# prabhask5/real-time-ray-tracing-engine

Hardware: AMD Instinct MI355X
Metric: Msamples/sec (W×H×spp) at 1080p, 8-bounce; 1/2/4/8 MI355X + CPU ref (higher is better)
Workload: dtype f64; 1 GPU; C2 three_spheres 1920x1080 spp64 depth8; scene=three_spheres, width=1920, height=1080, spp=64, max_depth=8, parallelism=1 GPU, device=gpu

## Files before the change

### __graft_entry__.py

```python
import os
import subprocess
import sys

ROOT = os.path.dirname(os.path.abspath(__file__))
PKG = os.path.join(ROOT, "real-time-ray-tracing-engine_amd")


def _make(path, *targets):
    jobs = "-j%d" % min(16, os.cpu_count() or 1)
    subprocess.run(["make", jobs, "-C", path] + list(targets), check=True)


def build():
    _make(PKG)
    _make(os.path.join(ROOT, "oracle"))
    _make(os.path.join(ROOT, "tests", "native"))
    _make(os.path.join(ROOT, "tests", "native"), "-f", "guides.mk")
    _make(os.path.join(ROOT, "tests", "native"), "-f", "temporal.mk")
    _make(os.path.join(ROOT, "tests", "native"), "-f", "temporal_variance.mk")
    _make(os.path.join(ROOT, "tests", "native"), "-f", "root_table.mk")
    _make(os.path.join(ROOT, "tests", "native"), "-f", "diffuse.mk")
    _make(os.path.join(ROOT, "tests", "native"), "-f", "unitv.mk")
    _make(os.path.join(ROOT, "tests", "native"), "-f", "refit.mk")
    _make(os.path.join(ROOT, "tests", "native"), "-f", "live.mk")
    _make(os.path.join(ROOT, "tests", "native"), "-f", "query.mk")
    _make(os.path.join(ROOT, "tests", "native"), "-f", "occlusion.mk")
    _make(os.path.join(ROOT, "tests", "native"), "-f", "lambert.mk")
    _make(os.path.join(ROOT, "tests", "native"), "-f", "radiance.mk")
    if os.path.isdir("/root/reference/src"):
        _make(os.path.join(ROOT, "oracle"), "ref")
    for p in (PKG, os.path.join(ROOT, "tests")):
        if p not in sys.path:
            sys.path.insert(0, p)
    import rtx
    from rtx.lib import load
    load()


def smoke():
    for p in (PKG, os.path.join(ROOT, "tests")):
        if p not in sys.path:
            sys.path.insert(0, p)
    import numpy as np
    import torch
    from rtx.render import Renderer, camera_frame
    from rtx.scene import load_scene
    import oracle_lib as O

    assert torch.cuda.is_available(), "smoke() needs a GPU"
    S = load_scene(os.path.join(PKG, "scenes", "cornell_fog.json"))
    cam = S.camera_desc(image_width=32, samples_per_pixel=4, max_depth=8)
    f = camera_frame(cam)
    with Renderer(S, device=0) as R:
        gpu = R.render(f, seed=42)
    ref = O.oracle_render(S, cam, O.MODE_COUNTER, 42)
    d = float(np.nanmax(np.abs(gpu - ref)))
    assert d <= 1e-4, "GPU vs oracle max |diff| %g" % d
    print("smoke ok: %dx%d cornell_fog, max |gpu - oracle| = %.3g" % (f.image_width, f.image_height, d))


if __name__ == "__main__":
    build()
    if len(sys.argv) > 1 and sys.argv[1] == "smoke":
        smoke()
```

### real-time-ray-tracing-engine_amd/csrc/rt_camq.h

```cpp
#ifndef RT_CAMQ_H
#define RT_CAMQ_H

#if defined(__HIPCC__)
#include <hip/hip_runtime.h>
#define RT_CAMQ_HD __host__ __device__
#else
#define RT_CAMQ_HD
#endif

namespace rtq {

constexpr int kBatch = 64;
constexpr int kBatches = 2;
constexpr int kEntries = kBatch * kBatches;
constexpr int kComps = 7;

RT_CAMQ_HD inline int camq_need(int next_item, int n_idle, int n_items) {
  const int e = next_item + n_idle;
  return e < n_items ? e : n_items;
}
RT_CAMQ_HD inline bool camq_generate(int gen_items, int need) { return gen_items < need; }
RT_CAMQ_HD inline int camq_batch(int gen_items) { return gen_items / kBatch; }
RT_CAMQ_HD inline int camq_write_entry(int gen_items, int lane) { return (gen_items & (kEntries - 1)) + lane; }
RT_CAMQ_HD inline int camq_read_entry(int item) { return item & (kEntries - 1); }
RT_CAMQ_HD inline bool camq_may_overwrite(int gen_items, int next_item) {
  return gen_items < kEntries || next_item >= gen_items - kBatch;
}

}
#endif
```

### real-time-ray-tracing-engine_amd/csrc/rt_kernel.hip

```cpp
#include <hip/hip_runtime.h>
#include <stdint.h>
#include <stdlib.h>

#include <algorithm>
#include <array>
#include <mutex>
#include <set>
#include <utility>

#include "rt_camq.h"
#include "rt_kernels.h"
#include "rt_lds_plan.h"
#include "rt_path.h"
#include "rt_plan.h"

namespace {

using namespace rtp;
#ifndef RT_REGEN_FLAT
#define RT_REGEN_FLAT 16
#endif
#define RT_REGEN_MIN(F) ((F) == F_FLAT ? RT_REGEN_FLAT : (((F) & ~F_BVH4) == 0 ? 16 : 1))
#ifndef RT_PARK_K
#define RT_PARK_K 48
// ... 164 lines not shown
      const bool whole = S.n_lds_nodes >= S.n_nodes;
      for (int k = threadIdx.x; k < n8; k += blockDim.x) {
        const int i = k / 10, j = k - 10 * (k / 10);
        const int a = j / 3, m = j - 3 * (j / 3);
        const int u = j == 9 ? 6 : (m == 1 ? 3 + a : a);
        uint2 v = src[8 * i + u];
        if (j == 9 && whole) {
          if ((int)v.x >= 0) v.x *= (unsigned)sizeof(DNodeL);
          if ((int)v.y >= 0) v.y *= (unsigned)sizeof(DNodeL);
        }
        dst[k] = v;
      }
    }
    if constexpr (PC) {
      if (S.lds_items_pc > 0) {
        const int ni = S.lds_items_pc * 2, ns = S.lds_spheres_pc * 4;
        const int4 *si = reinterpret_cast<const int4 *>(S.items);
        const int4 *ss = reinterpret_cast<const int4 *>(S.spheres);
        for (int k = threadIdx.x; k < ni; k += blockDim.x) prim_g[k] = si[k];
        for (int k = threadIdx.x; k < ns; k += blockDim.x) prim_g[ni + k] = ss[k];
      }
    }
    __syncthreads();
  }
  if constexpr ((F & F_NOISE) != 0) {
    if (S.lds_perlin) {
      const int4 *src = reinterpret_cast<const int4 *>(S.perlin);
      RT_LDS int4 *dst = (RT_LDS int4 *)perlin_lds();
      for (int k = threadIdx.x; k < (int)(sizeof(DPerlin) / 16); k += blockDim.x) dst[k] = src[k];
      __syncthreads();
    }
  }
  const int n_units = P.n_head * P.head_chunks + (P.n_local_tiles - P.n_head) * P.n_chunks;
  int unit = blockIdx.x * BW + wv;
  int *stk = stack_base + wv * S.stack_depth * 64 + lane;
  double *acc = &acc_lds[wv][0][0];
  Counters cnt{0, 0, 0, 0, 0, 0, 0, 0, 0, 0, 0, 0, 0, 0, 0};
  uint64_t cyc_regen = 0;
  const uint64_t t_start = STATS ? clk() : 0;
  uint32_t n_samples = 0, n_segments = 0, n_trips = 0;
  uint64_t m_single = 0, m_pair = 0;
  uint32_t v_prev = 0, m_prev = 0;
  bool have_prev = false;
  auto wave_max = [](uint32_t x) {
    for (int off = 32; off > 0; off >>= 1) x = max(x, (uint32_t)__shfl_xor((int)x, off));
    return x;
  };
  while (unit < n_units) {
#if RT_UNIT_TIMES
  const unsigned long long t_unit0 = __builtin_amdgcn_s_memrealtime();
#endif
  const DLaunch PU = launch_fields<PC>(P);
  const int head_units = PU.n_head * PU.head_chunks;
  const bool whole = PU.head_chunks == 1 && unit < PU.n_head;
  int local_tile, s_first, s_count;
  {
    const bool head = unit < head_units;
    const int nc = head ? PU.head_chunks : PU.n_chunks;
    const int cs = head ? (PU.sample_count + nc - 1) / nc : PU.chunk_strata;
    const int u = head ? unit : unit - head_units, q = u / nc, chunk = u - q * nc;
    local_tile = head ? q : PU.n_head + q;
    s_first = PU.sample_begin + chunk * cs;
    s_count = min(cs, PU.sample_count - chunk * cs);
  }
  local_tile = order_tile(PU, local_tile);
  if constexpr (STATS || COST) {
    if (lane == 0 && PU.tile_cost != nullptr)
      atomicSub(&PU.tile_cost[local_tile], (unsigned)__builtin_amdgcn_s_memrealtime());
  }
  const int tile = PU.tile_first + local_tile * PU.tile_stride;
  const int tx = tile % PU.tiles_x, ty = tile / PU.tiles_x;
  const int x0 = tx * 8, y0 = PU.row_begin + ty * 8;
  acc[lane * 3 + 0] = 0.0;
  acc[lane * 3 + 1] = 0.0;
  acc[lane * 3 + 2] = 0.0;

  const int n_items = 64 * max(0, s_count);
  int next_item = 0;
  constexpr bool kCamq = F == F_FLAT;
  [[maybe_unused]] int gen_items = 0;
  PathState ps;
  ps.active = false;
  Key key{P.seed_lo, P.seed_hi, 0, 0};
  constexpr int kPark = RT_PARK_MIN(F);
  [[maybe_unused]] double pk_closest = 0.0;
  [[maybe_unused]] int pk_best = -1;

  for (;;) {
    const uint64_t t_regen = STATS ? clk() : 0;
    for (;;) {
      unsigned long long idle = __ballot(!ps.active);
      if (idle == 0 || next_item >= n_items) break;
      if (__popcll(idle) < RT_REGEN_MIN(F) && ~idle != 0ull) break;
      if constexpr (kCamq) {
        static_assert(BW == 1, "the camera-ray queue is one wave's");
        __shared__ double camq[rtq::kComps][rtq::kEntries];
        const DCamera &Cr = C;
        const bool lens = !(Cr.defocus_angle <= 0);
        const int rank = (int)__builtin_amdgcn_mbcnt_hi((uint32_t)(idle >> 32), __builtin_amdgcn_mbcnt_lo((uint32_t)idle, 0u));
        const int item = next_item + rank;
        const int need = __builtin_amdgcn_readfirstlane(rtq::camq_need(next_item, __popcll(idle), n_items));
        while (rtq::camq_generate(gen_items, need)) {
          const DCamera Cg = camera_fields<true>(C);
          const int gk = __builtin_amdgcn_readfirstlane(s_first + rtq::camq_batch(gen_items));
          const int gi = x0 + (lane & 7), gj = y0 + (lane >> 3);
          const Key gkey{P.seed_lo, P.seed_hi, (uint32_t)(gj * Cg.W + gi), (uint32_t)gk};
          const Ray gr = camera_ray<RT_KB_F(F), RT_KCONST_MODE(F)>(Cg, gkey, gi, gj, gk);
          const int e = rtq::camq_write_entry(gen_items, lane);
          camq[0][e] = gr.d.x;
          camq[1][e] = gr.d.y;
          camq[2][e] = gr.d.z;
          camq[3][e] = gr.tm;
          if (lens) {
            camq[4][e] = gr.o.x;
            camq[5][e] = gr.o.y;
            camq[6][e] = gr.o.z;
          }
          gen_items += rtq::kBatch;
        }
        __builtin_amdgcn_fence(__ATOMIC_RELEASE, "wavefront");
        __builtin_amdgcn_wave_barrier();
        __builtin_amdgcn_fence(__ATOMIC_ACQUIRE, "wavefront");
        next_item += __popcll(idle);
        if (!ps.active && item < n_items) {
          int slot = item & 63;
          int i = x0 + (slot & 7), j = y0 + (slot >> 3);
          if (i < Cr.W && j < P.row_end) {
            const int e = rtq::camq_read_entry(item);
            ps.slot = slot;
            ps.sample = s_first + (item >> 6);
            key.pixel = (uint32_t)(j * Cr.W + i);
            key.sample = (uint32_t)ps.sample;
            ps.ray.d = v3(camq[0][e], camq[1][e], camq[2][e]);
            ps.ray.tm = camq[3][e];
            ps.ray.o = lens ? v3(camq[4][e], camq[5][e], camq[6][e]) : ld3(Cr.center);
            ps.T = v3(1.0, 1.0, 1.0);
            ps.bounce = 0;
            ps.active = Cr.max_depth > 0;
            if (STATS) n_samples++;
          }
        }
      } else {
        int rank = __popcll(idle & ((1ull << lane) - 1ull));
        int item = next_item + rank;
        next_item += __popcll(idle);
        if (!ps.active && item < n_items) {
          const DCamera &Cr = C;
          int slot = item & 63;
          int i = x0 + (slot & 7), j = y0 + (slot >> 3);
          if (i < Cr.W && j < P.row_end) {
            ps.slot = slot;
            ps.sample = s_first + (item >> 6);
            key.pixel = (uint32_t)(j * Cr.W + i);
            key.sample = (uint32_t)ps.sample;
            ps.ray = camera_ray<RT_KB_F(F), RT_KCONST_MODE(F)>(Cr, key, i, j, ps.sample);
            ps.T = v3(1.0, 1.0, 1.0);
            ps.bounce = 0;
            ps.active = Cr.max_depth > 0;
            if (STATS) n_samples++;
          }
        }
      }
    }
    if (STATS) cyc_regen += clk() - t_regen;
    if (__ballot(ps.active) == 0) break;
    if (STATS) n_trips++;
    uint32_t v_trace = 0;
    if constexpr (kPark > 0) {
      bool done = false;
      if (ps.active && pk_best < 0) {
        if (STATS) n_segments++;
        const uint64_t t0 = STATS ? clk() : 0;
        trace_closest<STATS, F, PC>(S, ps.ray, pk_closest, pk_best, stk, lnodes, cnt,
                                    (RT_LDS LeafPool *)&leaf_pool[0], lp);
        if (STATS && wave_once()) cnt.ctrace += clk() - t0;
        if (pk_best < 0) {
          ps.T = ps.T * ld3(C.bg);
          done = true;
        }
      }
      const bool parked = ps.active && pk_best >= 0;
      const bool wait = __popcll(__ballot(parked)) < kPark && next_item < n_items &&
                        __popcll(__ballot(!ps.active || done)) >= RT_REGEN_MIN(F);
      if (!wait && parked) {
        const uint64_t t1 = STATS ? clk() : 0;
        done = !shade_closest<STATS, F, PC, MS>(S, C, ps, key, pk_closest, pk_best, cnt, lp);
        if (STATS && wave_once()) cnt.cshade += clk() - t1;
        pk_best = -1;
      }
      if (done) {
        atomicAdd(&acc[ps.slot * 3 + 0], ps.T.x);
        atomicAdd(&acc[ps.slot * 3 + 1], ps.T.y);
        atomicAdd(&acc[ps.slot * 3 + 2], ps.T.z);
        ps.active = false;
      }
    } else if (ps.active) {
      if (STATS) n_segments++;
      const uint32_t nv0 = cnt.nodes;
      bool cont = segment<STATS, F, PC, MS>(
          S, C, ps, key, stk, lnodes, cnt, (RT_LDS LeafPool *)&leaf_pool[RT_LEAF_SHARE_F(F) ? wv : 0], lp);
      if (STATS) v_trace = cnt.nodes - nv0;
      if (!cont) {
        atomicAdd(&acc[ps.slot * 3 + 0], ps.T.x);
        atomicAdd(&acc[ps.slot * 3 + 1], ps.T.y);
        atomicAdd(&acc[ps.slot * 3 + 2], ps.T.z);
        ps.active = false;
      }
    }
    if (STATS) {
      const uint32_t m1 = wave_max(v_trace);
      m_single += m1;
      if (!have_prev) {
        v_prev = v_trace;
        m_prev = m1;
      } else {
        m_pair += wave_max(v_prev + v_trace);
      }
      have_prev = !have_prev;
    }
  }
  if (STATS && have_prev) {
    m_pair += m_prev;
// ... 164 lines not shown
```

### real-time-ray-tracing-engine_amd/csrc/rt_path.h

```cpp
#ifndef RT_PATH_H
#define RT_PATH_H
#include <math.h>
#include <stdint.h>

#include <array>
#include <utility>

#include "../../include/rt_api.h"
#include "rt_layout.h"

#if defined(__HIPCC__)
#include <hip/hip_runtime.h>
#define RT_HD __host__ __device__
#define RT_FI __forceinline__
#else
#define RT_HD
#define RT_FI inline
#endif
#if defined(__HIP_DEVICE_COMPILE__)
#define RT_LDS __attribute__((address_space(3)))
#else
#define RT_LDS
#endif

// ... 341 lines not shown
  for (int i = 0; i < 2; i++) {
    int pxi = P->px[(xi + i) & 255];
    double fi = i ? uu : 1 - uu, di = i ? u - 1 : u;
    for (int j = 0; j < 2; j++) {
      int pyj = P->py[(yi + j) & 255];
      double fj = j ? vv : 1 - vv, dj = j ? v - 1 : v;
      for (int k = 0; k < 2; k++) {
        const auto *g = P->rv[pxi ^ pyj ^ P->pz[(zi + k) & 255]];
        double fk = k ? ww : 1 - ww, dk = k ? w - 1 : w;
        acc += fi * fj * fk * (g[0] * di + g[1] * dj + g[2] * dk);
      }
    }
  }
  return acc;
}

using PerlinLds = DPerlin;
#if defined(__HIP__)
__device__ __forceinline__ const RT_LDS PerlinLds *perlin_lds() {
  __shared__ PerlinLds table;
  return (const RT_LDS PerlinLds *)&table;
}
#endif


template <unsigned F, MatSet MS = M_ANY>
RT_HD V3 tex_value(const DScene &S, int t, V3 p) {
  if constexpr (MS == M_DIFFUSE) return ld3(S.texs[t].color);
  for (int guard = 0; guard < 64; ++guard) {
    const DTex &T = S.texs[t];
    if (T.kind == RT_TEX_SOLID) return ld3(T.color);
    if (T.kind == RT_TEX_CHECKER) {
      const double inv = T.inv_scale;
      int xi = (int)floor(inv * p.x), yi = (int)floor(inv * p.y), zi = (int)floor(inv * p.z);
      t = ((xi + yi + zi) % 2 == 0) ? T.even : T.odd;
      continue;
    }
    if constexpr ((F & F_NOISE) != 0) {
      auto turb = [&](auto P) {
        double acc = 0.0, wgt = 1.0;
        V3 q = p;
#pragma unroll 1
        for (int i = 0; i < 7; i++) {
          acc += wgt * perlin_noise(P, q);
          wgt *= 0.5;
          q = v3(q.x * 2, q.y * 2, q.z * 2);
        }
        return acc;
      };
#if defined(__HIP_DEVICE_COMPILE__)
      const double acc = S.lds_perlin ? turb(perlin_lds()) : turb(&S.perlin[T.perlin]);
#else
      const double acc = turb(&S.perlin[T.perlin]);
#endif
      double f = 1 + sin_n(T.scale * p.z + 10 * fabs(acc));
      return f * v3(0.5, 0.5, 0.5);
    }
    break;
  }
  return v3(0, 0, 0);
}

template <bool MOVING = true>
RT_HD RT_FI V3 sphere_center(const DSphere &s, double tm) {
  if constexpr (!MOVING) return ld3(s.c0);
  return v3(s.c0[0] + tm * s.dir[0], s.c0[1] + tm * s.dir[1], s.c0[2] + tm * s.dir[2]);
}
RT_HD RT_FI double div_mk(double x, double b, double y) {
  const double q = x * y;
  const double r = fma(-q, b, x);
  return fma(r, y, q);
}
constexpr double kInvPi = 1.0 / kPi;

template <bool MOVING = true>
RT_HD RT_FI bool sphere_root(const DSphere &s, const Ray &r, double a, double tmin,
                                            double tmax, double &root, bool mk = false,
                                            double ya = 0.0) {
  V3 cc = sphere_center<MOVING>(s, r.tm);
  V3 oc = cc - r.o;
  double h = dot(r.d, oc);
  double c = len2(oc) - s.rr;
  double disc = h * h - a * c;
  if (disc < 0) return false;
  double sq = sqrt(disc);
  double t = mk ? div_mk(h - sq, a, ya) : (h - sq) / a;
  if (!(tmin < t && t < tmax)) {
    t = mk ? div_mk(h + sq, a, ya) : (h + sq) / a;
    if (!(tmin < t && t < tmax)) return false;
  }
  root = t;
  return true;
}
template <bool MOVING = true>
RT_HD RT_FI void sphere_record(const DSphere &s, const Ray &r, double t, int mat,
                                              Hit &h) {
  V3 cc = sphere_center<MOVING>(s, r.tm);
  h.t = t;
  h.p = at(r, t);
  V3 on = s.inv_r * (h.p - cc);
  h.front = dot(r.d, on) < 0;
  h.n = h.front ? on : -on;
  h.mat = mat;
}

#define RT_UNIFORM_LOADS_F(F) ((F) == F_FLAT)
#define RT_ROOT_TABLE_F(F) ((F) == F_FLAT)
RT_HD RT_FI double comp(V3 v, int a) { return a == 0 ? v.x : (a == 1 ? v.y : v.z); }
template <bool SEL = false>
RT_HD RT_FI bool quad_t_aa(const DQuad &q, const Ray &r, double tmin, double tmax, double &t) {
  const int k = q.aa & 3, i = (q.aa >> 2) & 3, j = (q.aa >> 4) & 3;
  const double nk = SEL ? comp(ld3(q.n), k) : q.n[k], wk = SEL ? comp(ld3(q.w), k) : q.w[k];
  const double Qi = SEL ? comp(ld3(q.Q), i) : q.Q[i], Qj = SEL ? comp(ld3(q.Q), j) : q.Q[j];
  const double vj = SEL ? comp(ld3(q.v), j) : q.v[j], ui = SEL ? comp(ld3(q.u), i) : q.u[i];
  const double denom = nk * comp(r.d, k);
  if (fabs(denom) < 1e-8 || fabs(denom) == kInf) return false;
  const double tt = (q.D - nk * comp(r.o, k)) / denom;
  if (!(tmin <= tt && tt <= tmax)) return false;
  const double pvi = (comp(r.o, i) + tt * comp(r.d, i)) - Qi;
  const double pvj = (comp(r.o, j) + tt * comp(r.d, j)) - Qj;
  const double ca = pvi * vj, cb = ui * pvj;
  const bool neg = (q.aa >> 6) & 1;
  const double alpha = wk * (neg ? -ca : ca);
  const double beta = wk * (neg ? -cb : cb);
  if (!(0 <= alpha && alpha <= 1) || !(0 <= beta && beta <= 1)) return false;
  t = tt;
  return true;
}
RT_HD RT_FI constexpr double comp_c(V3 v, int a) { return a == 0 ? v.x : (a == 1 ? v.y : v.z); }
template <int K, int I, int J>
RT_HD RT_FI bool quad_t_aa_c(const DQuad &q, const Ray &r, double tmin, double tmax, double &t) {
  constexpr bool neg = !((K + 1) % 3 == I);
  const double nk = q.n[K], wk = q.w[K], Qi = q.Q[I], Qj = q.Q[J], vj = q.v[J], ui = q.u[I];
  const double denom = nk * comp_c(r.d, K);
  if (fabs(denom) < 1e-8 || fabs(denom) == kInf) return false;
  const double tt = (q.D - nk * comp_c(r.o, K)) / denom;
  if (!(tmin <= tt && tt <= tmax)) return false;
  const double pvi = (comp_c(r.o, I) + tt * comp_c(r.d, I)) - Qi;
  const double pvj = (comp_c(r.o, J) + tt * comp_c(r.d, J)) - Qj;
  const double ca = pvi * vj, cb = ui * pvj;
  const double alpha = wk * (neg ? -ca : ca);
  const double beta = wk * (neg ? -cb : cb);
  if (!(0 <= alpha && alpha <= 1) || !(0 <= beta && beta <= 1)) return false;
  t = tt;
  return true;
}
RT_HD RT_FI bool quad_t_aa_u(const DQuad &q, const Ray &r, double tmin, double tmax, double &t) {
  switch (q.aa & 63) {
  case 0 | 1 << 2 | 2 << 4: return quad_t_aa_c<0, 1, 2>(q, r, tmin, tmax, t);
  case 0 | 2 << 2 | 1 << 4: return quad_t_aa_c<0, 2, 1>(q, r, tmin, tmax, t);
  case 1 | 2 << 2 | 0 << 4: return quad_t_aa_c<1, 2, 0>(q, r, tmin, tmax, t);
  case 1 | 0 << 2 | 2 << 4: return quad_t_aa_c<1, 0, 2>(q, r, tmin, tmax, t);
  case 2 | 0 << 2 | 1 << 4: return quad_t_aa_c<2, 0, 1>(q, r, tmin, tmax, t);
  default: return quad_t_aa_c<2, 1, 0>(q, r, tmin, tmax, t);
  }
}
template <bool SEL = false, bool UAX = false>
RT_HD RT_FI bool quad_t(const DQuad &q, const Ray &r, double tmin, double tmax,
                                       double &t) {
  if constexpr (UAX) {
    if (q.aa >= 0) return quad_t_aa_u(q, r, tmin, tmax, t);
  }
  if (q.aa >= 0) return quad_t_aa<SEL>(q, r, tmin, tmax, t);
  V3 n = ld3(q.n);
  double denom = dot(n, r.d);
  if (fabs(denom) < 1e-8) return false;
// ... 563 lines not shown
        d.dir[k] = L.dir[k];
      }
      d.inv_r = L.inv_r;
      d.rr = L.rr;
      return d;
    }
  }
  return S.spheres[i];
}

template <bool STATS, unsigned F, bool LP = false>
RT_HD RT_FI bool trace_tail(const DScene &S, const Ray &r, Hit &h, const Key &key,
                                           uint32_t bounce, double closest, int best,
                                           Counters &cnt, const LdsPrims &lp = LdsPrims{}) {
  const double tmin = 0.001;
  constexpr bool kFlat = (F & F_FLAT) != 0;
  bool best_full = false;
  if constexpr ((F & F_MEDIA) != 0) {
    const uint64_t t0 = STATS ? clk() : 0;
    constexpr bool kFma = !kFlat;
    const RayF<kFma> q = ray_f32<kFma>(r);
    const float tmin32 = f32_dn(tmin);
    float cl32 = f32_up(closest);
    int best_m = -1;
    for (int m = 0; m < S.n_mitems; ++m) {
      if (slab(q, S.mbox + 6 * m, S.mbox + 6 * m + 3, tmin32, cl32) == __builtin_huge_valf())
        continue;
      if (STATS) cnt.other++;
      double tm_hit;
      int box_path;
      const bool mh = medium_t<RT_KB_F(F)>(S, S.mitems[m], r, tmin, closest, key, bounce, tm_hit, box_path);
      if (STATS) {
        cnt.mbox += box_path >= 0;
        cnt.mbox_fb += box_path == 0;
      }
      if (mh) {
        closest = tm_hit;
        cl32 = f32_up(closest);
        best_m = m;
      }
    }
    if (best_m >= 0) {
      medium_record(S, S.mitems[best_m], r, closest, h);
      best = best_m;
      best_full = true;
    }
    if (STATS && wave_once()) cnt.cmedia += clk() - t0;
  }
  if (best < 0) return false;
  auto item_record = [&](auto mv) {
    const DItem it = load_item<LP>(S, lp, best);
    Ray lr = r;
    if constexpr ((F & F_XFORM) != 0) {
      if (it.xf_count) lr = to_local(S, it.xf_first, it.xf_count, r);
    }
    if (it.kind == I_SPHERE)
      sphere_record<decltype(mv)::value>(load_sphere<LP>(S, lp, it.idx), lr, closest, it.mat, h);
    else
      quad_record(S.quads[it.idx], lr, closest, it.mat, h);
    if constexpr ((F & F_XFORM) != 0) {
      if (it.xf_count) to_world(S, it.xf_first, it.xf_count, h);
    }
  };
  if (!best_full) {
    if constexpr (RT_ROOT_TABLE_F(F)) {
      if (S.n_roots) {
        const DRoot R = S.roots[best];
        DSphere s;
        s.c0[0] = R.test.c0[0], s.c0[1] = R.test.c0[1], s.c0[2] = R.test.c0[2];
        s.inv_r = R.inv_r;
        sphere_record<false>(s, r, closest, R.mat, h);
        return true;
      }
    }
    if constexpr (kFlat) {
      if (S.static_spheres) {
        item_record(UTag<false>{});
        return true;
      }
    }
    item_record(UTag<true>{});
  }
  return true;
}


template <bool STATS, unsigned F, bool LP = false, bool ROOTS = false>
RT_HD RT_FI bool trace(const DScene &S, const Ray &r, Hit &h, const Key &key,
                                      uint32_t bounce, int *stk, const RT_LDS DNode *lnodes,
                                      Counters &cnt, RT_LDS LeafPool *pool = nullptr,
                                      const LdsPrims &lp = LdsPrims{}, double *closest_out = nullptr,
                                      int *best_out = nullptr) {
  const double tmin = 0.001;
  double closest = kInf;
  int best = -1;
  const double a = len2(r.d);
  const double ya = 1.0 / a;
  constexpr bool kFlat = (F & F_FLAT) != 0;
  constexpr bool kBoxes = !kFlat || (F & F_MEDIA) != 0;
  constexpr bool kFma = !kFlat;
  RayF<kFma> q{};
  float tmin32 = 0.0f;
  float cl32 = __builtin_huge_valf();
  if constexpr (kBoxes) {
    q = ray_f32<kFma>(r);
    tmin32 = f32_dn(tmin);
  }

  auto item_root_t = [&](auto uniform, auto mv, int ii, const Ray &rr, double ra, double ry,
                         double tmax, double &t) -> bool {
    constexpr bool U = decltype(uniform)::value && RT_UNIFORM_LOADS_F(F);
    constexpr bool MV = decltype(mv)::value;
    const DItem it = U ? ldu<U>(S.items, ii) : load_item<LP>(S, lp, ii);
    Ray lr = rr;
    double al = ra;
    bool local = false;
    if constexpr ((F & F_XFORM) != 0) {
      if (it.xf_count) {
        lr = to_local<U>(S, it.xf_first, it.xf_count, rr);
        al = len2(lr.d);
        local = true;
      }
    }
    if (it.kind == I_SPHERE) {
      if (STATS) cnt.spheres++;
      const double yl = local ? 1.0 / al : ry;
      return sphere_root<MV>(U ? ldu<U>(S.spheres, it.idx) : load_sphere<LP>(S, lp, it.idx), lr,
                             al, tmin, tmax, t, true, yl);
    }
    if (STATS) cnt.quads++;
    constexpr bool UA = decltype(uniform)::value;
    if constexpr (U) return quad_t<true, UA>(ldu<true>(S.quads, it.idx), lr, tmin, tmax, t);
    return quad_t<false, UA>(S.quads[it.idx], lr, tmin, tmax, t);
  };
  [[maybe_unused]] auto item_root = [&](int ii, const Ray &rr, double ra, double ry, double tmax,
                                        double &t) -> bool {
    return item_root_t(UTag<false>{}, UTag<true>{}, ii, rr, ra, ry, tmax, t);
  };
  auto test_item_m = [&](auto uniform, auto mv, int ii) {
    if (STATS) cnt.wleaf += wave_once();
    double t;
    const bool hit = item_root_t(uniform, mv, ii, r, a, ya, closest, t);
    if (hit) {
      closest = t;
      if constexpr (kBoxes) cl32 = f32_up_c(closest);
      best = ii;
    }
  };
  [[maybe_unused]] auto test_item = [&](auto uniform, int ii) { test_item_m(uniform, UTag<true>{}, ii); };

  [[maybe_unused]] constexpr bool kShare = RT_LEAF_SHARE_F(F);
#if defined(__HIP_DEVICE_COMPILE__)
  auto leaf_share = [&](int &ln_, int &lf_) {
    constexpr int kPrev = 1 << 26;
    const int lane = (int)__lane_id();
    const uint64_t below = (1ull << lane) - 1ull;
    const uint64_t ex = __ballot(1);
    int pre = 0, tot = 0;
#pragma unroll
    for (int b = 0; b < 3; ++b) {
      const uint64_t m = __ballot((ln_ >> b) & 1);
      pre += __popcll(m & below) << b;
      tot += __popcll(m) << b;
    }
    const int nx = __popcll(ex), rk = __popcll(ex & below);
    unsigned long long cbits = (unsigned long long)__double_as_longlong(closest);
    int ckey = kPrev;
    pool->bt[lane] = cbits;
    pool->bk[lane] = kPrev;
    for (int base = 0; base < tot; base += nx) {
      if (STATS) cnt.wleaf += wave_once();
      for (int k = base > pre ? base - pre : 0; k < ln_ && pre + k < base + nx; ++k)
        pool->tab[pre + k - base] = ((lf_ + k) << 6) | lane;
      __builtin_amdgcn_wave_barrier();
      const int w = base + rk;
      int o = lane, ii = 0;
      if (w < tot) {
        const int e = pool->tab[rk];
        o = e & 63;
        ii = e >> 6;
      }
      Ray ro;
      ro.o = v3(__shfl(r.o.x, o), __shfl(r.o.y, o), __shfl(r.o.z, o));
      ro.d = v3(__shfl(r.d.x, o), __shfl(r.d.y, o), __shfl(r.d.z, o));
      ro.tm = __shfl(r.tm, o);
      const double ra = __shfl(a, o), ry = __shfl(ya, o);
      bool hit = false;
      double t = 0.0;
      unsigned long long tb = 0;
      int key = 0;
      if (w < tot) {
        const double tmax = __longlong_as_double((long long)pool->bt[o]);
        hit = item_root(ii, ro, ra, ry, tmax, t);
        tb = (unsigned long long)__double_as_longlong(t);
        key = S.items[ii].kind == I_SPHERE ? kPrev + 1 + ii : kPrev - 1 - ii;
        if (hit)
          __hip_atomic_fetch_min(&pool->bt[o], tb, __ATOMIC_RELAXED, __HIP_MEMORY_SCOPE_WAVEFRONT);
      }
      __builtin_amdgcn_wave_barrier();
      if (pool->bt[lane] != cbits) pool->bk[lane] = 0x7fffffff;
      __builtin_amdgcn_wave_barrier();
      const bool at_min = hit && pool->bt[o] == tb;
      if (at_min)
        __hip_atomic_fetch_min(&pool->bk[o], key, __ATOMIC_RELAXED, __HIP_MEMORY_SCOPE_WAVEFRONT);
      __builtin_amdgcn_wave_barrier();
      if (at_min && pool->bk[o] == key) pool->bi[o] = ii;
      __builtin_amdgcn_wave_barrier();
      const unsigned long long nb = pool->bt[lane];
      const int nk = pool->bk[lane];
      if (nb != cbits || nk != ckey) {
        cbits = nb;
        ckey = nk;
        closest = __longlong_as_double((long long)nb);
        best = pool->bi[lane];
        if constexpr (kBoxes) cl32 = f32_up_c(closest);
      }
      __builtin_amdgcn_wave_barrier();
    }
    lf_ += ln_;
    ln_ = 0;
  };
#endif

  if constexpr (kFlat) {
    if (RT_ROOT_TABLE_F(F) && S.n_roots) {
      const int n = S.n_roots;
      auto load_test = [&](int ii) { return ldu<true>(&S.roots[ii].test, 0); };
      auto test_root = [&](const DRootTest &e, int ii) {
        if (STATS) {
          cnt.wleaf += wave_once();
          cnt.spheres++;
        }
        DSphere s;
        s.c0[0] = e.c0[0], s.c0[1] = e.c0[1], s.c0[2] = e.c0[2];
        s.rr = e.rr;
        double t;
        if (sphere_root<false>(s, r, a, tmin, closest, t, true, ya)) {
#if defined(__HIP_DEVICE_COMPILE__)
          asm volatile("");
#endif
          closest = t;
          if constexpr (kBoxes) cl32 = f32_up_c(closest);
          best = ii;
        }
      };
      for (int ii = 0; ii < n; ++ii) test_root(load_test(ii), ii);
    } else if (S.static_spheres) {
      for (int ii = 0; ii < S.n_root_items; ++ii) test_item_m(UTag<true>{}, UTag<false>{}, ii);
    } else {
      for (int ii = 0; ii < S.n_root_items; ++ii) test_item_m(UTag<true>{}, UTag<true>{}, ii);
    }
  } else {
    int *top = stk;
    auto push = [&](int e) {
      *top = e;
      top += 64;
    };
    auto pop = [&]() -> int {
      if (top == stk) return -1;
      top -= 64;
      return *top;
    };
    [[maybe_unused]] PlaneOff po{};
    if constexpr (kFma)
      po = (F & F_BVH4) == 0 ? plane_offsets_l(q) : plane_offsets<(F & F_BVH4) ? 4 : 2>(q);
    int cur;
    int lf = 0, ln = 0;
    if (S.root_is_leaf) {
      cur = -1;
      ln = S.n_root_items;
    } else {
      cur = 0;
    }
    for (;;) {
      if constexpr ((F & F_BVH4) != 0) {
        const RT_LDS DNode4 *lnodes4 = (const RT_LDS DNode4 *)lnodes;
        const DNode4 *nodes4 = (const DNode4 *)S.nodes;
        while (cur >= 0) {
          if (STATS) cnt.wnode += wave_once();
          if (wave_none(ln == 0)) break;
          if (STATS) cnt.nodes++;
          float tn[4];
          int en[4];
          if constexpr (kFma) {
            NodePlanes<4> pl;
            if (cur < S.n_lds_nodes)
              load_planes<4>(pl, (const RT_LDS char *)lnodes4, cur * (int)sizeof(DNode4), po);
            else
              load_planes<4>(pl, (const char *)nodes4, cur * (int)sizeof(DNode4), po);
            bool hh[4];
            slab_planes<4>(q, pl, tmin32, cl32, tn, hh);
#pragma unroll
            for (int c = 0; c < 4; ++c) {
              en[c] = pl.en[c];
              if (en[c] == -1 || !hh[c]) tn[c] = __builtin_huge_valf();
            }
          } else {
            DNode4 N;
            if (cur < S.n_lds_nodes) {
              const RT_LDS DNode4 &L = lnodes4[cur];
#pragma unroll
              for (int a = 0; a < 3; ++a)
#pragma unroll
                for (int c = 0; c < 4; ++c) {
                  N.lo[a][c] = L.lo[a][c];
                  N.hi[a][c] = L.hi[a][c];
                }
#pragma unroll
              for (int c = 0; c < 4; ++c) N.entry[c] = L.entry[c];
            } else {
              N = nodes4[cur];
            }
#pragma unroll
            for (int c = 0; c < 4; ++c) {
              const float lo[3] = {N.lo[0][c], N.lo[1][c], N.lo[2][c]};
              const float hi[3] = {N.hi[0][c], N.hi[1][c], N.hi[2][c]};
              en[c] = N.entry[c];
              tn[c] = en[c] == -1 ? __builtin_huge_valf() : slab(q, lo, hi, tmin32, cl32);
            }
          }
          auto cswap = [&](int x, int y) {
            const bool sw = tn[y] < tn[x];
            const float tx = tn[x], ty = tn[y];
            const int ex = en[x], ey = en[y];
            tn[x] = sw ? ty : tx;
            tn[y] = sw ? tx : ty;
            en[x] = sw ? ey : ex;
            en[y] = sw ? ex : ey;
          };
// ... 43 lines not shown
                N.entry[1] = L.entry[1];
              } else {
                N = S.nodes[cur];
              }
              slab_hit2(q, N, tmin32, cl32, tn0, tn1, h0, h1);
              e0 = N.entry[0];
              e1 = N.entry[1];
            }
            if (h0 && h1) {
              const bool first0 = tn0 <= tn1;
              push(first0 ? e1 : e0);
              cur = first0 ? e0 : e1;
            } else if (h0 || h1) {
              cur = h0 ? e0 : e1;
            } else {
              cur = pop();
            }
            if (cur < -1 && ln == 0) {
              lf = (~cur) >> 3;
              ln = (~cur) & 7;
              cur = pop();
            }
          }
        };
        if (kFma && S.n_lds_nodes >= S.n_nodes)
          walk(UTag<true>{});
        else
          walk(UTag<false>{});
      }
#if defined(__HIP_DEVICE_COMPILE__)
      if constexpr (kShare) {
        if (__ballot(ln > 0) == 0) break;
        int mx = 1;
#pragma unroll
        for (int k = 2; k <= 7; ++k)
          if (__ballot(ln >= k) != 0) mx = k;
        int tot = 0;
#pragma unroll
        for (int b = 0; b < 3; ++b) tot += __popcll(__ballot((ln >> b) & 1)) << b;
        const int nx = __popcll(__ballot(1));
        if ((tot + nx - 1) / nx < mx) {
          leaf_share(ln, lf);
        } else {
          while (ln > 0) {
            const int ii = lf;
            ++lf;
            --ln;
            test_item(UTag<false>{}, ii);
          }
        }
      } else
#endif
      {
        if (ln == 0) break;
        while (ln > 0) {
          const int ii = lf;
          ++lf;
          --ln;
          test_item(UTag<false>{}, ii);
        }
      }
      if (cur < -1) {
        lf = (~cur) >> 3;
        ln = (~cur) & 7;
        cur = pop();
      }
    }
  }
  if constexpr (ROOTS) {
    *closest_out = closest;
    *best_out = best;
    return best >= 0;
  } else {
    return trace_tail<STATS, F, LP>(S, r, h, key, bounce, closest, best, cnt, lp);
  }
}
template <bool STATS, unsigned F, bool LP = false>
RT_HD RT_FI void trace_closest(const DScene &S, const Ray &r, double &closest, int &best, int *stk,
                               const RT_LDS DNode *lnodes, Counters &cnt,
                               RT_LDS LeafPool *pool = nullptr, const LdsPrims &lp = LdsPrims{}) {
  Hit h;
  trace<STATS, F, LP, true>(S, r, h, Key{}, 0u, stk, lnodes, cnt, pool, lp, &closest, &best);
}

template <bool STATS>
RT_HD double lights_pdf(const DScene &S, V3 org, V3 dir, Counters &cnt) {
  double sum = 0.0;
  for (int i = 0; i < S.n_lights; ++i) {
    const DLight L = S.lights[i];
    Ray lr = to_local(S, L.xf_first, L.xf_count, Ray{org, dir, 0.0});
    double p = 0.0;
    if (L.kind == I_SPHERE) {
      if (STATS) cnt.light++;
      const DSphere &s = S.spheres[L.idx];
      double t;
      if (sphere_root(s, lr, len2(lr.d), 0.001, kInf, t)) {
        V3 c0 = v3(s.c0[0] + 0 * s.dir[0], s.c0[1] + 0 * s.dir[1], s.c0[2] + 0 * s.dir[2]);
        double dist2 = len2(c0 - lr.o);
        double ctm = sqrt(1 - s.rr / dist2);
        double sa = 2 * kPi * (1 - ctm);
        p = 1 / sa;
      }
    } else if (L.kind == I_QUAD) {
      if (STATS) cnt.light++;
      const DQuad &q = S.quads[L.idx];
      double t;
      if (quad_t<false, true>(q, lr, 0.001, kInf, t)) {
        V3 n = ld3(q.n);
        V3 fn = dot(lr.d, n) < 0 ? n : -n;
        double d2 = t * t * len2(lr.d);
        double cosine = fabs(dot(lr.d, fn) / sqrt(len2(lr.d)));
        p = d2 / (cosine * q.area);
      }
    }
    sum += L.weight * p;
  }
  return sum;
}

template <int KC = 0, bool SC = false>
RT_HD V3 lights_random(const DScene &S, V3 org, double upick, double r1, double r2,
                       double sp1 = 0.0, double cp1 = 0.0) {
  int k = S.n_lights - 1;
  for (int i = 0; i < S.n_lights; ++i)
    if (upick < S.lights[i].cum) {
      k = i;
      break;
    }
  const DLight L = S.lights[k];
  V3 p = to_local(S, L.xf_first, L.xf_count, Ray{org, v3(0, 0, 0), 0.0}).o;
  V3 d;
  if (L.kind == I_SPHERE) {
    const DSphere &s = S.spheres[L.idx];
    V3 c0 = v3(s.c0[0] + 0 * s.dir[0], s.c0[1] + 0 * s.dir[1], s.c0[2] + 0 * s.dir[2]);
    V3 dir = c0 - p;
    double d2 = len2(dir);
    V3 w = unitv(dir);
    V3 a = (fabs(w.x) > 0.9) ? v3(0, 1, 0) : v3(1, 0, 0);
    V3 vv = unitv(cross(w, a));
    V3 uu = cross(w, vv);
    double z = 1 + r2 * (sqrt(1 - s.rr / d2) - 1);
    double sphi = sp1, cphi = cp1;
    if constexpr (!SC) sincos_2pi<KC>(r1, sphi, cphi);
    double x = cphi * sqrt(1 - z * z);
    double y = sphi * sqrt(1 - z * z);
    d = ((x * uu) + (y * vv)) + (z * w);
  } else if (L.kind == I_QUAD) {
    const DQuad &q = S.quads[L.idx];
    V3 pt = (ld3(q.Q) + (r1 * ld3(q.u))) + (r2 * ld3(q.v));
    d = pt - p;
  } else {
    d = v3(1, 0, 0);
  }
  for (int c = L.xf_count - 1; c >= 0; --c) {
    const DXform X = S.xforms[L.xf_first + c];
    if (X.kind == X_ROTATE_Y) d = rot_out(X.a, X.b, d);
  }
  return d;
}

struct PathState {
  Ray ray;
  V3 T;
  uint32_t bounce;
  int slot;
  int sample;
// ... 283 lines not shown
```

Baseline: 37050 Msamples/s.

## Trace camera rays against root table during batched generation with precomputed origin terms

When camera rays for a pinhole camera are generated in the per-wave queue, each batch is now traced against the root sphere table right away, with full lane occupancy. The closest hit and index are stored in the queue, so lanes that pick up the item start already parked with a hit, and misses write background colour directly. Per-sphere origin terms (oc and c) for the camera centre are precomputed once into LDS so camera-ray tests skip recomputing them. This is meant to cut divergent, partly filled trace passes for primary rays. It adds LDS use, queue storage for two more fields, and extra logic in the refill loop.

```diff
diff --git a/__graft_entry__.py b/__graft_entry__.py
--- a/__graft_entry__.py
+++ b/__graft_entry__.py
@@ -27,6 +27,7 @@
     _make(os.path.join(ROOT, "tests", "native"), "-f", "occlusion.mk")
     _make(os.path.join(ROOT, "tests", "native"), "-f", "lambert.mk")
     _make(os.path.join(ROOT, "tests", "native"), "-f", "radiance.mk")
+    _make(os.path.join(ROOT, "tests", "native"), "-f", "root_origin.mk")
     if os.path.isdir("/root/reference/src"):
         _make(os.path.join(ROOT, "oracle"), "ref")
     for p in (PKG, os.path.join(ROOT, "tests")):
diff --git a/profiles/batch_hist.py b/profiles/batch_hist.py
--- /dev/null
+++ b/profiles/batch_hist.py
@@ -0,0 +1,43 @@
+import ctypes as C
+import json
+import os
+import sys
+
+ROOT = os.path.dirname(os.path.dirname(os.path.abspath(__file__)))
+sys.path.insert(0, os.path.join(ROOT, "real-time-ray-tracing-engine_amd"))
+from rtx.lib import load
+from rtx.render import Renderer, camera_frame
+from rtx.scene import load_scene
+
+TEST_VALU = 48
+ORIGIN_VALU = 9
+N_ROOTS = 3
+SQ_INSTS_VALU = 1862e6
+
+L = load()
+S = load_scene(os.path.join(ROOT, "real-time-ray-tracing-engine_amd", "scenes", "three_spheres.json"))
+f = camera_frame(S.camera_desc(image_width=1920, samples_per_pixel=64, max_depth=8))
+with Renderer(S) as R:
+    st = R.stats(f, seed=42)
+    h = (C.c_uint64 * 32)()
+    L.rtk_trace_hist.argtypes = [C.c_void_p]
+    assert L.rtk_trace_hist(h) == 0
+h = list(h)
+print("STATS", json.dumps({k: v for k, v in sorted(st.items()) if not k.startswith("cyc_")}))
+print("# trace passes of C2 (1920x1080, 64 strata, depth 8; STATS instance: the schedule is the parent's)")
+print("# lanes traced | passes | camera-ray lanes | bounce-ray lanes")
+for b in range(8):
+    print("%2d-%2d %10d %12d %12d" % (8 * b + 1, 8 * b + 8, h[b], h[8 + b], h[16 + b]))
+passes, cam, bnc = sum(h[:8]), sum(h[8:16]), sum(h[16:24])
+print("# passes %d (trips %d, without a trace pass %d), lanes traced %d = camera %d + bounce %d (segments %d, samples %d)" % (
+    passes, st["wave_trips"], h[24], cam + bnc, cam, bnc, st["segments"], st["samples"]))
+print("# lane use of the trace %.3f; camera rays are %.1f %% of the traced lanes" % (
+    (cam + bnc) / (64.0 * max(1, passes)), 100.0 * cam / max(1, cam + bnc)))
+batches, shades = st["samples"] // 64, st["wave_shade_iters"]
+after = batches + shades
+part1 = (passes - after) * N_ROOTS * TEST_VALU
+part2 = batches * N_ROOTS * ORIGIN_VALU
+print("# model, part 1: passes %d -> at most %d batches + %d shade passes = %d: -%.0f M VALU (%.1f %% of %.0f M)" % (
+    passes, batches, shades, after, part1 / 1e6, 100.0 * part1 / SQ_INSTS_VALU, SQ_INSTS_VALU / 1e6))
+print("# model, part 2: %d batches x %d roots x %d operations: -%.0f M VALU (%.1f %%)" % (
+    batches, N_ROOTS, ORIGIN_VALU, part2 / 1e6, 100.0 * part2 / SQ_INSTS_VALU))
diff --git a/real-time-ray-tracing-engine_amd/csrc/rt_camq.h b/real-time-ray-tracing-engine_amd/csrc/rt_camq.h
--- a/real-time-ray-tracing-engine_amd/csrc/rt_camq.h
+++ b/real-time-ray-tracing-engine_amd/csrc/rt_camq.h
@@ -14,6 +14,8 @@
 constexpr int kBatches = 2;
 constexpr int kEntries = kBatch * kBatches;
 constexpr int kComps = 7;
+constexpr int kClosest = 4;
+constexpr int kBest = 5;
 
 RT_CAMQ_HD inline int camq_need(int next_item, int n_idle, int n_items) {
   const int e = next_item + n_idle;
diff --git a/real-time-ray-tracing-engine_amd/csrc/rt_kernel.hip b/real-time-ray-tracing-engine_amd/csrc/rt_kernel.hip
--- a/real-time-ray-tracing-engine_amd/csrc/rt_kernel.hip
+++ b/real-time-ray-tracing-engine_amd/csrc/rt_kernel.hip
@@ -270,6 +270,24 @@
   PathState ps;
   ps.active = false;
   Key key{P.seed_lo, P.seed_hi, 0, 0};
+  [[maybe_unused]] bool gen_trace = false, org_tab = false;
+  [[maybe_unused]] const RT_LDS RootOrigin *root_org = nullptr;
+  if constexpr (kCamq) {
+    __shared__ RootOrigin root_org_lds[kRootOriginMax > 0 ? kRootOriginMax : 1];
+    root_org = (const RT_LDS RootOrigin *)&root_org_lds[0];
+    gen_trace = RT_ROOT_TABLE_F(F) && n_items > rtq::kBatch && C.defocus_angle <= 0 && S.n_roots > 0;
+    org_tab = gen_trace && S.n_roots <= kRootOriginMax;
+    if (org_tab) {
+      const DCamera Co = camera_fields<true>(C);
+      for (int ii = 0; ii < S.n_roots; ++ii) {
+        const RootOrigin q = root_origin(ldu<true>(&S.roots[ii].test, 0), ld3(Co.center));
+        if (lane == 0) root_org_lds[ii] = q;
+      }
+      __builtin_amdgcn_fence(__ATOMIC_RELEASE, "wavefront");
+      __builtin_amdgcn_wave_barrier();
+      __builtin_amdgcn_fence(__ATOMIC_ACQUIRE, "wavefront");
+    }
+  }
   constexpr int kPark = RT_PARK_MIN(F);
   [[maybe_unused]] double pk_closest = 0.0;
   [[maybe_unused]] int pk_best = -1;
@@ -303,6 +321,20 @@
             camq[4][e] = gr.o.x;
             camq[5][e] = gr.o.y;
             camq[6][e] = gr.o.z;
+          } else if (gen_trace) {
+            double g_closest = 0.0;
+            int g_best = -1;
+            if (gi < Cg.W && gj < P.row_end && Cg.max_depth > 0) {
+              if (STATS) n_segments++;
+              const uint64_t t0 = STATS ? clk() : 0;
+              if (org_tab)
+                trace_closest_roots<STATS, true>(S, root_org, gr, g_closest, g_best, cnt);
+              else
+                trace_closest_roots<STATS, false>(S, root_org, gr, g_closest, g_best, cnt);
+              if (STATS && wave_once()) cnt.ctrace += clk() - t0;
+            }
+            camq[rtq::kClosest][e] = g_closest;
+            camq[rtq::kBest][e] = __longlong_as_double((long long)g_best);
           }
           gen_items += rtq::kBatch;
         }
@@ -321,11 +353,26 @@
             key.sample = (uint32_t)ps.sample;
             ps.ray.d = v3(camq[0][e], camq[1][e], camq[2][e]);
             ps.ray.tm = camq[3][e];
-            ps.ray.o = lens ? v3(camq[4][e], camq[5][e], camq[6][e]) : ld3(Cr.center);
             ps.T = v3(1.0, 1.0, 1.0);
             ps.bounce = 0;
-            ps.active = Cr.max_depth > 0;
             if (STATS) n_samples++;
+            if (!gen_trace) {
+              ps.ray.o = lens ? v3(camq[4][e], camq[5][e], camq[6][e]) : ld3(Cr.center);
+              ps.active = Cr.max_depth > 0;
+            } else if (Cr.max_depth > 0) {
+              ps.ray.o = ld3(Cr.center);
+              const int eb = (int)__double_as_longlong(camq[rtq::kBest][e]);
+              if (eb >= 0) {
+                pk_closest = camq[rtq::kClosest][e];
+                pk_best = eb;
+                ps.active = true;
+              } else {
+                const V3 sky = ps.T * ld3(C.bg);
+                atomicAdd(&acc[slot * 3 + 0], sky.x);
+                atomicAdd(&acc[slot * 3 + 1], sky.y);
+                atomicAdd(&acc[slot * 3 + 2], sky.z);
+              }
+            }
           }
         }
       } else {
diff --git a/real-time-ray-tracing-engine_amd/csrc/rt_path.h b/real-time-ray-tracing-engine_amd/csrc/rt_path.h
--- a/real-time-ray-tracing-engine_amd/csrc/rt_path.h
+++ b/real-time-ray-tracing-engine_amd/csrc/rt_path.h
@@ -447,6 +447,29 @@
   double h = dot(r.d, oc);
   double c = len2(oc) - s.rr;
   double disc = h * h - a * c;
+  if (disc < 0) return false;
+  double sq = sqrt(disc);
+  double t = mk ? div_mk(h - sq, a, ya) : (h - sq) / a;
+  if (!(tmin < t && t < tmax)) {
+    t = mk ? div_mk(h + sq, a, ya) : (h + sq) / a;
+    if (!(tmin < t && t < tmax)) return false;
+  }
+  root = t;
+  return true;
+}
+struct RootOrigin {
+  V3 oc;
+  double c;
+};
+RT_HD RT_FI RootOrigin root_origin(const DRootTest &e, V3 o) {
+  V3 cc = ld3(e.c0);
+  V3 oc = cc - o;
+  return RootOrigin{oc, len2(oc) - e.rr};
+}
+RT_HD RT_FI bool sphere_root_origin(const RootOrigin &q, const Ray &r, double a, double tmin, double tmax,
+                                    double &root, bool mk = false, double ya = 0.0) {
+  double h = dot(r.d, q.oc);
+  double disc = h * h - a * q.c;
   if (disc < 0) return false;
   double sq = sqrt(disc);
   double t = mk ? div_mk(h - sq, a, ya) : (h - sq) / a;
@@ -1176,6 +1199,35 @@
     item_record(UTag<true>{});
   }
   return true;
+}
+
+template <bool STATS, bool ORG>
+RT_HD RT_FI bool root_table_test(const DScene &S, const RT_LDS RootOrigin *tab, int ii, const Ray &r, double a,
+                                 double ya, double tmin, double &closest, int &best, Counters &cnt) {
+  if (STATS) {
+    cnt.wleaf += wave_once();
+    cnt.spheres++;
+  }
+  double t;
+  bool hit;
+  if constexpr (ORG) {
+    const RootOrigin q = tab[ii];
+    hit = sphere_root_origin(q, r, a, tmin, closest, t, true, ya);
+  } else {
+    const DRootTest e = ldu<true>(&S.roots[ii].test, 0);
+    DSphere s;
+    s.c0[0] = e.c0[0], s.c0[1] = e.c0[1], s.c0[2] = e.c0[2];
+    s.rr = e.rr;
+    hit = sphere_root<false>(s, r, a, tmin, closest, t, true, ya);
+  }
+  if (hit) {
+#if defined(__HIP_DEVICE_COMPILE__)
+    asm volatile("");
+#endif
+    closest = t;
+    best = ii;
+  }
+  return hit;
 }
 
 
@@ -1319,26 +1371,10 @@
   if constexpr (kFlat) {
     if (RT_ROOT_TABLE_F(F) && S.n_roots) {
       const int n = S.n_roots;
-      auto load_test = [&](int ii) { return ldu<true>(&S.roots[ii].test, 0); };
-      auto test_root = [&](const DRootTest &e, int ii) {
-        if (STATS) {
-          cnt.wleaf += wave_once();
-          cnt.spheres++;
+      for (int ii = 0; ii < n; ++ii)
+        if (root_table_test<STATS, false>(S, nullptr, ii, r, a, ya, tmin, closest, best, cnt)) {
+          if constexpr (kBoxes) cl32 = f32_up_c(closest);
         }
-        DSphere s;
-        s.c0[0] = e.c0[0], s.c0[1] = e.c0[1], s.c0[2] = e.c0[2];
-        s.rr = e.rr;
-        double t;
-        if (sphere_root<false>(s, r, a, tmin, closest, t, true, ya)) {
-#if defined(__HIP_DEVICE_COMPILE__)
-          asm volatile("");
-#endif
-          closest = t;
-          if constexpr (kBoxes) cl32 = f32_up_c(closest);
-          best = ii;
-        }
-      };
-      for (int ii = 0; ii < n; ++ii) test_root(load_test(ii), ii);
     } else if (S.static_spheres) {
       for (int ii = 0; ii < S.n_root_items; ++ii) test_item_m(UTag<true>{}, UTag<false>{}, ii);
     } else {
@@ -1548,6 +1584,20 @@
   Hit h;
   trace<STATS, F, LP, true>(S, r, h, Key{}, 0u, stk, lnodes, cnt, pool, lp, &closest, &best);
 }
+#ifndef RT_ROOT_ORIGIN_MAX
+#define RT_ROOT_ORIGIN_MAX 4
+#endif
+constexpr int kRootOriginMax = RT_ROOT_ORIGIN_MAX;
+template <bool STATS, bool ORG>
+RT_HD RT_FI void trace_closest_roots(const DScene &S, const RT_LDS RootOrigin *tab, const Ray &r, double &closest,
+                                     int &best, Counters &cnt) {
+  const double tmin = 0.001;
+  closest = kInf;
+  best = -1;
+  const double a = len2(r.d);
+  const double ya = 1.0 / a;
+  for (int ii = 0; ii < S.n_roots; ++ii) root_table_test<STATS, ORG>(S, tab, ii, r, a, ya, tmin, closest, best, cnt);
+}
 
 template <bool STATS>
 RT_HD double lights_pdf(const DScene &S, V3 org, V3 dir, Counters &cnt) {
diff --git a/real-time-ray-tracing-engine_amd/host/rtx_batch_check.cpp b/real-time-ray-tracing-engine_amd/host/rtx_batch_check.cpp
--- /dev/null
+++ b/real-time-ray-tracing-engine_amd/host/rtx_batch_check.cpp
@@ -0,0 +1,159 @@
+#include <stdint.h>
+#include <stdio.h>
+#include <stdlib.h>
+#include <string.h>
+
+#include <vector>
+
+#include "../csrc/rt_camq.h"
+
+static uint64_t rng_state;
+static uint32_t rnd() {
+  uint64_t z = (rng_state += 0x9E3779B97F4A7C15ull);
+  z = (z ^ (z >> 30)) * 0xBF58476D1CE4E5B9ull;
+  z = (z ^ (z >> 27)) * 0x94D049BB133111EBull;
+  return (uint32_t)((z ^ (z >> 31)) >> 32);
+}
+
+#define FAIL(...)                 \
+  do {                            \
+    fprintf(stderr, __VA_ARGS__); \
+    fprintf(stderr, "\n");        \
+    return 1;                     \
+  } while (0)
+
+struct Entry {
+  int item = -1;
+  bool inside = false;
+  bool hit = false;
+};
+
+int main(int argc, char **argv) {
+  if (argc != 6) {
+    fprintf(stderr, "usage: rtx_batch_check N_ITEMS THRESHOLD K SEED mixed|allmiss|allhit|lens\n");
+    return 2;
+  }
+  const int n_items = atoi(argv[1]), threshold = atoi(argv[2]), park_k = atoi(argv[3]);
+  rng_state = strtoull(argv[4], nullptr, 10);
+  const char *mode = argv[5];
+  const bool lens = !strcmp(mode, "lens"), allmiss = !strcmp(mode, "allmiss"), allhit = !strcmp(mode, "allhit");
+  if (!lens && !allmiss && !allhit && strcmp(mode, "mixed")) return 2;
+  if (n_items < 0 || n_items % rtq::kBatch != 0 || threshold < 1 || threshold > 64 || park_k < 1 || park_k > 64)
+    return 2;
+  const int max_depth = 8;
+
+  Entry ring[rtq::kEntries];
+  std::vector<int> settled(n_items, 0), handed(n_items, 0), outside(n_items, 0);
+  bool active[64] = {}, parked[64] = {};
+  int bounce[64] = {};
+  int next_item = 0, gen_items = 0;
+  long trips = 0, passes = 0, max_passes = 0, n_hits = 0, n_misses = 0, n_outside = 0, n_waits = 0, n_shades = 0;
+  bool waited = false;
+  const long trip_cap = 64L * (n_items + 64) * (max_depth + 2);
+  for (;; ++trips) {
+    if (trips > trip_cap) FAIL("the loop does not end: %ld trips, head %d of %d", trips, next_item, n_items);
+    int took = 0;
+    long trip_passes = 0;
+    for (;;) {
+      uint64_t idle = 0;
+      for (int l = 0; l < 64; ++l)
+        if (!active[l]) idle |= 1ull << l;
+      if (idle == 0 || next_item >= n_items) break;
+      const int n_idle = __builtin_popcountll(idle);
+      if (n_idle < threshold && ~idle != 0ull) break;
+      const int need = rtq::camq_need(next_item, n_idle, n_items);
+      while (rtq::camq_generate(gen_items, need)) {
+        if (!rtq::camq_may_overwrite(gen_items, next_item))
+          FAIL("batch at %d would overwrite unpopped items (head %d)", gen_items, next_item);
+        const uint32_t p_hit = rnd() % 257;
+        for (int l = 0; l < 64; ++l) {
+          Entry &e = ring[rtq::camq_write_entry(gen_items, l)];
+          if (e.item >= next_item) FAIL("entry of unpopped item %d overwritten", e.item);
+          e.item = gen_items + l;
+          e.inside = rnd() % 16 != 0;
+          e.hit = !lens && e.inside && (allhit || (!allmiss && rnd() % 256 < p_hit));
+        }
+        gen_items += rtq::kBatch;
+      }
+      const int head = next_item;
+      next_item += n_idle;
+      for (int l = 0; l < 64; ++l) {
+        const int rank = __builtin_popcountll(idle & ((1ull << l) - 1ull));
+        const int item = head + rank;
+        if (active[l] || item >= n_items) continue;
+        if (parked[l]) FAIL("idle lane %d holds a parked hit", l);
+        const Entry &e = ring[rtq::camq_read_entry(item)];
+        if (e.item != item) FAIL("lane %d reads item %d from an entry that holds %d", l, item, e.item);
+        ++took;
+        if (!e.inside) {
+          ++outside[item];
+          ++n_outside;
+        } else if (lens) {
+          ++handed[item];
+          active[l] = true;
+          bounce[l] = 0;
+        } else if (e.hit) {
+          ++handed[item];
+          ++n_hits;
+          active[l] = parked[l] = true;
+          bounce[l] = 0;
+        } else {
+          ++settled[item];
+          ++n_misses;
+        }
+      }
+      if (next_item <= head) FAIL("a refill pass at head %d took nothing", head);
+      ++passes;
+      ++trip_passes;
+    }
+    if (trip_passes > max_passes) max_passes = trip_passes;
+    if (waited && took == 0) FAIL("trip %ld follows a waiting trip and its refill takes no item (head %d of %d)", trips, next_item, n_items);
+    bool any = false;
+    for (int l = 0; l < 64; ++l) any = any || active[l];
+    if (!any) break;
+    bool done[64] = {};
+    int traced = 0, shaded = 0;
+    for (int l = 0; l < 64; ++l)
+      if (active[l] && !parked[l]) {
+        ++traced;
+        const bool camera = bounce[l] == 0;
+        if (camera && !lens) FAIL("lane %d traces a camera ray in the path loop", l);
+        const bool hit = camera ? (allhit || (!allmiss && rnd() % 2 != 0)) : rnd() % 4 != 0;
+        if (hit) parked[l] = true;
+        else {
+          done[l] = true;
+          if (camera) ++n_misses;
+        }
+        if (camera && hit) ++n_hits;
+      }
+    int n_parked = 0, n_free = 0;
+    for (int l = 0; l < 64; ++l) {
+      n_parked += active[l] && parked[l];
+      n_free += !active[l] || done[l];
+    }
+    const bool wait = n_parked < park_k && next_item < n_items && n_free >= threshold;
+    if (!wait)
+      for (int l = 0; l < 64; ++l)
+        if (active[l] && parked[l]) {
+          ++shaded;
+          parked[l] = false;
+          ++bounce[l];
+          if (bounce[l] >= max_depth || rnd() % 8 == 0) done[l] = true;
+        }
+    n_waits += wait;
+    n_shades += shaded > 0;
+    if (took == 0 && traced == 0 && shaded == 0)
+      FAIL("trip %ld takes no item, traces no lane and shades none (head %d of %d)", trips, next_item, n_items);
+    for (int l = 0; l < 64; ++l)
+      if (done[l]) active[l] = false;
+    waited = wait;
+  }
+  if (next_item < n_items || gen_items != n_items) FAIL("ended at head %d, %d generated, of %d", next_item, gen_items, n_items);
+  for (int k = 0; k < n_items; ++k) {
+    const int n = settled[k] + handed[k] + outside[k];
+    if (n != 1) FAIL("item %d: settled %d, handed %d, outside %d", k, settled[k], handed[k], outside[k]);
+  }
+  printf("OK items %d hits %ld misses %ld outside %ld trips %ld passes %ld max_passes %ld waits %ld shades %ld\n", n_items,
+         n_hits, n_misses, n_outside, trips, passes, max_passes, n_waits, n_shades);
+  return 0;
+}
```

New measurement: 39230 Msamples/s (median of 6 runs). +5.9%, better.
